# vniclas/VFM-Registration

Hardware: AMD Instinct MI355X
Metric: registrations/sec (20k<->200k pts, 384-D) (higher is better)
Workload: dtype fp6 (MX e2m3) coarse pass (scaled MFMA, fp32 scores + bounds from measured residuals) + int8 rescan (exact integer scores) + f32 refinement + f64 exact decision / f64 RANSAC

## Files before the change

include/vfmreg_debug.h:

```cpp
#ifndef VFMREG_DEBUG_H
#define VFMREG_DEBUG_H

#include "vfmreg.h"

#ifdef __cplusplus
extern "C" {
#endif

int vfm_prof_events_create(void **start, void **stop);
int vfm_prof_arm(void *start, void *stop);
int vfm_prof_elapsed_ms(void *start, void *stop, float *ms_host);
int vfm_prof_events_destroy(void *start, void *stop);

int vfm_debug_last_coarse_kernel(char *buf_host, int cap);
int vfm_debug_coarse_kernel_names(char *buf_host, int cap);

int vfm_debug_search_plan(int records, int d, int64_t n, int64_t m, int gated, char *buf_host, int cap);

int vfm_debug_coarse_plan(int records, int d, int64_t n, int64_t m, int gated, int inner_product, int row_bias, int compute_units,
                          char *buf_host, int cap);

enum vfm_debug_prepare_entry {
    VFM_PREP_ENTRY_PREPARE = 0,
    VFM_PREP_ENTRY_PREPARE2,
    VFM_PREP_ENTRY_GATED,
    VFM_PREP_ENTRY_GATED_P,
    VFM_PREP_ENTRY_GATED_Z,
    VFM_PREP_ENTRY_GATED_T,
    VFM_PREP_ENTRY_PERM,
    VFM_PREP_ENTRY_ONESHOT
};
int vfm_debug_prepare_plan(int entry, int schedule, int d, int64_t rows1, int dtype1, int64_t rows2, int dtype2, int zero, char *buf_host,
                           int cap);

int vfm_debug_match_stats(void *ws, int64_t n, int64_t m, int32_t *out64_host);
int vfm_debug_voxel_trace(void *ws, int64_t n, int64_t *out_host);
int vfm_debug_i8_rows(const void *prepared, int64_t rows, int d, int8_t *q8_host, float *step_host,
                      float *err_host, float *gerr_host);
int vfm_debug_mx6_rows(const void *prepared, int64_t rows, int d, float *v6_host, float *err_host, float *gerr_host);
int vfm_debug_mx6_half_err(const void *prepared, int64_t rows, int d, float *errh_host, float *gerrh_host);
int vfm_debug_ransac_counts(const void *ws, int64_t c_max, int32_t n_iter, int32_t *out_host);
#define VFM_DEBUG_RANSAC_CAND_MAX 2048
int vfm_debug_ransac_state(const void *ws, int64_t c_max, int32_t n_iter, int32_t *n_lo_host, int32_t *n_hi_host, double *r_lo_host,
                           double *r_hi_host, int32_t *sel_host, double *rstar_host, int32_t *list_host, double *fit_host,
                           double *rmse_host, int32_t *hyp_host);

int vfm_debug_vit_workspace_layout(const vfm_vit_config *cfg, int B, int64_t *offsets_host, int64_t *bytes_host);

int vfm_debug_vit_plan(const vfm_vit_config *cfg, int B, int W, int compute_units, char *buf_host, int cap);

int vfm_debug_l2_narrow_slices(int64_t n, int64_t m);
int vfm_debug_l2_narrow_evals(const void *ws, int64_t *out2_host);

#ifdef __cplusplus
}
#endif
#endif
```

vfm-registration_amd/csrc/config.cpp:

```cpp
#include "common.h"
#include "config.h"

#include <string.h>

#include <new>

struct vfm_config {
    VfmConfig c;
};

static const VfmConfig k_factory{};
static thread_local const VfmConfig* t_bound = nullptr;

const VfmConfig& vfm_cfg() { return t_bound ? *t_bound : k_factory; }

namespace {
struct Field {
    const char* name;
    int VfmConfig::*p;
};
const Field k_fields[] = {
    {"coarse_slices", &VfmConfig::force_slices},     {"match_stats", &VfmConfig::match_stats},
    {"i8_min_queries", &VfmConfig::i8_min_queries},  {"prep_grid", &VfmConfig::prep_grid},
    {"ransac_exact_only", &VfmConfig::ransac_exact_only}, {"ransac_fused", &VfmConfig::ransac_fused},
    {"coarse_qsets", &VfmConfig::coarse_qsets},      {"seed_units", &VfmConfig::seed_units},
    {"select_variant", &VfmConfig::select_variant},  {"mx6_t4", &VfmConfig::mx6_t4},
    {"mx6_tune", &VfmConfig::mx6_tune},
    {"mx6_ns3", &VfmConfig::mx6_ns3},                {"prep_form", &VfmConfig::prep_form},
    {"finish_short", &VfmConfig::finish_short},      {"rescan_rows", &VfmConfig::rescan_rows},
    {"half_noi8", &VfmConfig::half_noi8},            {"rescore_block", &VfmConfig::rescore_block},
    {"vit_preprocess_patch", &VfmConfig::vit_preprocess_patch}, {"vit_xcd", &VfmConfig::vit_xcd},
    {"vit_cfg_narrow", &VfmConfig::vit_cfg_narrow},  {"vit_cfg_wide", &VfmConfig::vit_cfg_wide},
    {"vit_wpw", &VfmConfig::vit_wpw},                {"vit_hot_a", &VfmConfig::vit_hot_a},
    {"vit_wide_tile", &VfmConfig::vit_wide_tile},    {"vit_lds_shape", &VfmConfig::vit_lds_shape},
    {"vit_att_lds_min", &VfmConfig::vit_att_lds_min}, {"vit_lds_min_wg", &VfmConfig::vit_lds_min_wg},
    {"vit_astat_min", &VfmConfig::vit_astat_min},    {"vit_astat_two", &VfmConfig::vit_astat_two},
    {"vit_astat_nw", &VfmConfig::vit_astat_nw},      {"vit_fused_qkv", &VfmConfig::vit_fused_qkv},
    {"vit_trace_fused", &VfmConfig::vit_trace_fused},  {"vit_fused_mlp", &VfmConfig::vit_fused_mlp},
    {"voxel_replay2", &VfmConfig::voxel_replay2},    {"voxel_one_launch", &VfmConfig::voxel_small},
    {"voxel_trace", &VfmConfig::voxel_trace},        {"voxel_grid_ppt", &VfmConfig::voxel_grid_ppt},
};

const char* const k_trace_buffer = "vit_trace_buffer";

void set_coarse_variant(VfmConfig& c, int v) {
    if (v == 60 || v == 61) { c.rescan_rows = v == 61 ? 1 : 0; return; }
    if (v == 50 || v == 51) { c.finish_short = v == 51 ? 1 : 0; return; }
    if (v >= 40 && v <= 44) { c.prep_form = v == 44 ? 4 : v == 43 ? 3 : v == 41 ? 1 : 0; return; }
    if (v == 32 || v == 33) { c.mx6_ns3 = v == 33 ? 1 : 0; return; }
    if (v == 30 || v == 31) { c.mx6_t4 = v == 30 ? 1 : 0; return; }
    c.seed_units = v == 7 ? 0 : 1;
    if (v == 7) v = 0;
    c.select_variant = v == 20 ? 1 : (v == 21 ? 2 : 0);
    if (v == 20 || v == 21) v = 0;
    c.coarse_qsets = v;
}
void set_voxel_small(VfmConfig& c, int on) {
    if (on == 2 || on == 3) c.voxel_replay2 = on == 3;
    else if (on >= 10 && on <= 10 + 64) c.voxel_grid_ppt = on - 10;
    else if (on == 100 || on == 101) c.voxel_trace = on - 100;
    else c.voxel_small = on;
}
}

VFM_EXPORT int vfm_config_create(vfm_config_t** out) {
    VFM_CHECK_ARG(out, "config_create: null pointer");
    *out = new (std::nothrow) vfm_config();
    if (!*out) return vfm_fail(VFM_EINVAL, "config_create: out of memory");
    return VFM_OK;
}
VFM_EXPORT int vfm_config_destroy(vfm_config_t* cfg) {
    if (cfg && t_bound == &cfg->c) t_bound = nullptr;
    delete cfg;
    return VFM_OK;
}
VFM_EXPORT int vfm_config_use(const vfm_config_t* cfg) {
    t_bound = cfg ? &cfg->c : nullptr;
    return VFM_OK;
}
VFM_EXPORT int vfm_config_set(vfm_config_t* cfg, const char* key, int64_t value) {
    VFM_CHECK_ARG(cfg && key, "config_set: null pointer");
    if ((!strcmp(key, "coarse_variant") && value == 42) || (!strcmp(key, "prep_form") && value == 2))
        return vfm_fail(VFM_EINVAL, "config_set: %s %lld (fp6 operand preparation by width) has been removed", key, (long long)value);
    if (!strcmp(key, "rescore_block") && value != 64 && value != 256)
        return vfm_fail(VFM_EINVAL, "config_set: rescore_block %lld (a workgroup of match_rescore_kernel owns 64 or 256 queries)", (long long)value);
    if (!strcmp(key, "coarse_variant")) { set_coarse_variant(cfg->c, (int)value); return VFM_OK; }
    if (!strcmp(key, "voxel_small")) { set_voxel_small(cfg->c, (int)value); return VFM_OK; }
    if (!strcmp(key, k_trace_buffer)) { cfg->c.vit_astat_dbg = reinterpret_cast<unsigned long long*>((uintptr_t)value); return VFM_OK; }
    for (const Field& f : k_fields)
        if (!strcmp(key, f.name)) {
            cfg->c.*(f.p) = (int)value;
            return VFM_OK;
        }
    return vfm_fail(VFM_EINVAL, "config_set: unknown key '%s'", key);
}
VFM_EXPORT int vfm_config_get(const vfm_config_t* cfg, const char* key, int64_t* value) {
    VFM_CHECK_ARG(key && value, "config_get: null pointer");
    const VfmConfig& c = cfg ? cfg->c : vfm_cfg();
    if (!strcmp(key, k_trace_buffer)) { *value = (int64_t)(uintptr_t)c.vit_astat_dbg; return VFM_OK; }
    for (const Field& f : k_fields)
        if (!strcmp(key, f.name)) {
            *value = c.*(f.p);
            return VFM_OK;
        }
    return vfm_fail(VFM_EINVAL, "config_get: unknown key '%s'", key);
}
```

vfm-registration_amd/csrc/config.h:

```cpp
#pragma once

struct VfmConfig {
    int force_slices = 0;
    int coarse_qsets = 0;
    int seed_units = 1;
    int select_variant = 0;
    int mx6_t4 = 1;
    int mx6_ns3 = 1;
    int prep_form = 3;
    int finish_short = 0;
    int half_noi8 = 1;
    int rescore_block = 0;
    int rescan_rows = 1;
    int mx6_tune = 0;
    int match_stats = 0;
    int i8_min_queries = 0;
    int prep_grid = -1;
    int ransac_exact_only = 0;
    int ransac_fused = 2;
    int vit_preprocess_patch = 1, vit_xcd = 1, vit_cfg_narrow = 108, vit_cfg_wide = 108, vit_wpw = 0, vit_hot_a = 0, vit_wide_tile = 0,
        vit_lds_shape = 23, vit_att_lds_min = 1, vit_lds_min_wg = 256, vit_astat_min = 0, vit_astat_two = 1, vit_astat_nw = 0,
        vit_trace_fused = 0,
        vit_fused_mlp = 0,
        vit_fused_qkv = 0;
    unsigned long long* vit_astat_dbg = nullptr;
    int voxel_replay2 = 1, voxel_small = 1, voxel_trace = 0, voxel_grid_ppt = 0;
};

const VfmConfig& vfm_cfg();
```

vfm-registration_amd/csrc/ransac.hip:

```cpp
#include <string.h>

#include <atomic>
#include <vector>

#include "../../include/vfmreg_debug.h"
#include "common.h"
#include "rot3.h"

namespace {

__device__ __forceinline__ void philox4x32_10(uint32_t c0, uint32_t c1, uint32_t c2, uint32_t c3, uint32_t k0,
                                              uint32_t k1, uint32_t out[4]) {
    const uint32_t M0 = 0xD2511F53u, M1 = 0xCD9E8D57u, W0 = 0x9E3779B9u, W1 = 0xBB67AE85u;
#pragma unroll
    for (int r = 0; r < 10; ++r) {
        const uint32_t hi0 = __umulhi(M0, c0), lo0 = M0 * c0;
        const uint32_t hi1 = __umulhi(M1, c2), lo1 = M1 * c2;
        const uint32_t n0 = hi1 ^ c1 ^ k0;
        const uint32_t n1 = lo1;
        const uint32_t n2 = hi0 ^ c3 ^ k1;
        const uint32_t n3 = lo0;
        c0 = n0; c1 = n1; c2 = n2; c3 = n3;
        k0 += W0; k1 += W1;
    }
    out[0] = c0; out[1] = c1; out[2] = c2; out[3] = c3;
}

__device__ bool kabsch_rows(const double* A, const double* B, const double* w, int64_t n, double denom_eps,
                            double T[12]) {
    double ma[3] = {0.0, 0.0, 0.0}, mb[3] = {0.0, 0.0, 0.0}, sw = 0.0;
    for (int64_t i = 0; i < n; ++i) {
        const double wi = w ? w[i] : 1.0;
        sw = sw + wi;
#pragma unroll
        for (int c = 0; c < 3; ++c) {
            ma[c] = ma[c] + wi * A[i * 3 + c];
            mb[c] = mb[c] + wi * B[i * 3 + c];
        }
    }
// ... 431 lines not shown
    __shared__ double red[6][1024];
    __shared__ double cen[6];
    const int64_t C = count_dev ? min(*count_dev, c_max) : c_max;
    if (threadIdx.x == 0) {
        sel->F = 0;
        sel->count = 0;
        sel->Rbits = 0x7FF0000000000000ull;
        sel->overflow = 0;
        sel->unsure = 0;
        sel->done = 0;
    }
    for (int64_t i = threadIdx.x; i < C; i += 1024) {
        int64_t a = corres[2 * i], b = corres[2 * i + 1];
        if (bad_out && (a < 0 || a >= ns || b < 0 || b >= nt)) {
            *bad_out = 1;
            a = b = 0;
        }
#pragma unroll
        for (int c = 0; c < 3; ++c) {
            pts[6 * i + c] = src[3 * a + c];
            pts[6 * i + 3 + c] = tgt[3 * b + c];
        }
    }
    __threadfence();
    __syncthreads();
    ransac_center_body(pts, C, stats, pts32, red, cen);
}

struct CoarseHyp {
    int32_t n_lo, n_hi;
    double r_lo, r_hi;
};

__global__ __launch_bounds__(64) void ransac_moment_kernel(const double* __restrict__ pts, const RansacStats* __restrict__ stats,
                                                           const int64_t* __restrict__ count_dev, int64_t c_max,
                                                           double max_d2, int32_t n_iter, uint64_t seed,
                                                           CoarseHyp* __restrict__ out, SelectState* __restrict__ sel, int rfuse) {
    const int64_t C = count_dev ? min(*count_dev, c_max) : c_max;
    const int lane = threadIdx.x;
    const int32_t h = (int32_t)(blockIdx.x * 64 + lane);
    CoarseHyp o = CoarseHyp{0, -1, 0.0, 0.0};
    bool unsure = false, sure_live = false;
    if (C >= 3 && h < n_iter) {
        double T[12];
        if (sample_T(pts, C, (uint32_t)h, seed, T)) {
            const double u = 1.1102230246251565e-16;
            double tau[3], taumax = 0.0, tt = 0.0, tabs = 0.0, rmax = 0.0;
#pragma unroll
            for (int r = 0; r < 3; ++r) {
                tau[r] = (T[4 * r + 3] + ((T[4 * r] * stats->cs[0] + T[4 * r + 1] * stats->cs[1]) + T[4 * r + 2] * stats->cs[2])) -
                         stats->cq[r];
                taumax = fmax(taumax, fabs(tau[r]));
                tt += tau[r] * tau[r];
                tabs = fmax(tabs, fabs(T[4 * r + 3]));
#pragma unroll
                for (int c = 0; c < 3; ++c) rmax = fmax(rmax, fabs(T[4 * r + c]));
            }
            const double reach = 4.01 * stats->M + taumax;
            const bool sure = (rmax <= 1.001) && (max_d2 > 0.0) && (3.0 * reach * reach * 1.001 < max_d2);
            if (!sure) {
                unsure = true;
            } else {
                const double* S = stats->Sss;
                double q1 = 0.0, rk = 0.0, t4 = 0.0;
#pragma unroll
                for (int a = 0; a < 3; ++a) {
                    const double x = T[4 * a], y = T[4 * a + 1], z = T[4 * a + 2];
                    q1 += (x * (S[0] * x + S[1] * y + S[2] * z) + y * (S[1] * x + S[3] * y + S[4] * z)) +
                          z * (S[2] * x + S[4] * y + S[5] * z);
                    rk += (x * stats->K[3 * a] + y * stats->K[3 * a + 1]) + z * stats->K[3 * a + 2];
                    t4 += tau[a] * (((x * stats->sbar[0] + y * stats->sbar[1]) + z * stats->sbar[2]) - stats->kbar[a]);
                }
                const double Cd = (double)C;
// ... 401 lines not shown
                sr[0] = sr[w];
                sh[0] = sh[w];
            }
        double T[12] = {1, 0, 0, 0, 0, 1, 0, 0, 0, 0, 1, 0};
        if (sh[0] >= 0) sample_T(pts, C, (uint32_t)sh[0], seed, T);
        for (int k = 0; k < 12; ++k) {
            T_out[k] = T[k];
            Ts[k] = T[k];
        }
        T_out[12] = 0.0;
        T_out[13] = 0.0;
        T_out[14] = 0.0;
        T_out[15] = 1.0;
        *fitness_out = (sh[0] >= 0) ? sf[0] : 0.0;
        *rmse_out = (sh[0] >= 0) ? sr[0] : 0.0;
        *best_hyp_out = sh[0];
    }
    __syncthreads();
    if (!mask) return;
    const bool have = sh[0] >= 0;
    double T[12];
#pragma unroll
    for (int k = 0; k < 12; ++k) T[k] = Ts[k];
    for (int64_t i = threadIdx.x; i < c_max; i += 1024) {
        uint8_t m = 0;
        if (i < C && have) {
            const double* p = pts + 6 * i;
            m = (err2(T, p[0], p[1], p[2], p[3], p[4], p[5]) < max_d2) ? 1 : 0;
        }
        mask[i] = m;
    }
}

__global__ __launch_bounds__(64) void ransac_exact_list_kernel(const double* __restrict__ pts,
                                                               const int64_t* __restrict__ count_dev, int64_t c_max,
                                                               double max_d2, int32_t n_iter, uint64_t seed,
                                                               const int32_t* __restrict__ list,
                                                               const SelectState* __restrict__ sel,
                                                               HypScore* __restrict__ best_out) {
    __shared__ __attribute__((aligned(16))) double d2s[EXACT_CHUNK];
    const int64_t C = count_dev ? min(*count_dev, c_max) : c_max;
    const int lane = threadIdx.x;
    HypScore res;
    res.fit = 0.0;
    res.rmse = 0.0;
    res.hyp = -1;
    const int ncand = sel->overflow ? 0 : min(sel->count, CAND_MAX);
    if ((int)blockIdx.x < ncand && C >= 3) {
        const int32_t h = list[blockIdx.x];
        double T[12];
        if (sample_T(pts, C, (uint32_t)h, seed, T)) {
            int64_t good = 0;
            double e2 = 0.0;
            for (int64_t base = 0; base < C; base += EXACT_CHUNK) {
                const int cnt = (int)min((int64_t)EXACT_CHUNK, C - base);
                __builtin_amdgcn_wave_barrier();
                int mine = 0;
                for (int i = lane; i < cnt; i += 64) {
                    const double* p = pts + 6 * (base + i);
                    const double d2 = err2(T, p[0], p[1], p[2], p[3], p[4], p[5]);
                    const bool in = d2 < max_d2;
                    mine += in ? 1 : 0;
                    d2s[i] = in ? d2 : 0.0;
                }
#pragma unroll
                for (int off = 32; off >= 1; off >>= 1) mine += __shfl_xor(mine, off);
                good += mine;
                __builtin_amdgcn_wave_barrier();
                int i = 0;
                if (cnt >= 32) {
                    double va[16], vb[16];
#pragma unroll
                    for (int u = 0; u < 16; ++u) va[u] = d2s[u];
                    for (; i + 48 <= cnt; i += 32) {
#pragma unroll
                        for (int u = 0; u < 16; ++u) vb[u] = d2s[i + 16 + u];
#pragma unroll
                        for (int u = 0; u < 16; ++u) e2 = e2 + va[u];
#pragma unroll
                        for (int u = 0; u < 16; ++u) va[u] = d2s[i + 32 + u];
#pragma unroll
                        for (int u = 0; u < 16; ++u) e2 = e2 + vb[u];
                    }
#pragma unroll
                    for (int u = 0; u < 16; ++u) e2 = e2 + va[u];
                    i += 16;
                }
                for (; i < cnt; ++i) e2 = e2 + d2s[i];
            }
            if (good > 0) {
                res.fit = (double)good / (double)C;
                res.rmse = sqrt(e2 / (double)good);
                res.hyp = h;
            }
        }
    }
    if (lane == 0) best_out[blockIdx.x] = res;
}

struct RansacWs {
    double* pts;
    float* pts32;
    RansacStats* stats;
    CoarseHyp* hyps;
    int32_t* list;
    SelectState* sel;
    HypScore* block_best;
    size_t bytes;
};
inline RansacWs carve_ransac(void* p, int64_t c_max, int32_t n_iter) {
    VfmCarver c(p);
    RansacWs w;
    w.pts = c.take<double>((size_t)(c_max > 0 ? c_max : 1) * 6);
    w.pts32 = c.take<float>((size_t)(c_max > 0 ? c_max : 1) * 6 + 4);
    w.stats = c.take<RansacStats>(1);
    w.hyps = c.take<CoarseHyp>((size_t)n_iter);
    w.list = c.take<int32_t>(CAND_MAX);
    w.sel = c.take<SelectState>(1);
    w.block_best = c.take<HypScore>((size_t)(n_iter + 63) / 64 + CAND_MAX + 1);
    w.bytes = c.used();
    return w;
}


}


VFM_EXPORT int vfm_debug_ransac_counts(const void* ws, int64_t c_max, int32_t n_iter, int32_t* out_host) {
    VFM_CHECK_ARG(ws && out_host && c_max >= 0 && n_iter > 0, "ransac_counts: bad arguments");
    RansacWs w = carve_ransac(const_cast<void*>(ws), c_max, n_iter);
// ... 13 lines not shown
    RansacWs w = carve_ransac(const_cast<void*>(ws), c_max, n_iter);
    SelectState s;
    VFM_CHECK_HIP(hipMemcpy(&s, w.sel, sizeof(s), hipMemcpyDeviceToHost));
    if (sel_host) {
        sel_host[0] = s.F;
        sel_host[1] = s.count;
        sel_host[2] = s.overflow;
        sel_host[3] = s.unsure;
    }
    if (rstar_host) memcpy(rstar_host, &s.Rbits, sizeof(double));
    if (n_lo_host || n_hi_host || r_lo_host || r_hi_host) {
        std::vector<CoarseHyp> hy((size_t)n_iter);
        VFM_CHECK_HIP(hipMemcpy(hy.data(), w.hyps, sizeof(CoarseHyp) * hy.size(), hipMemcpyDeviceToHost));
        for (int32_t h = 0; h < n_iter; ++h) {
            if (n_lo_host) n_lo_host[h] = hy[h].n_lo;
            if (n_hi_host) n_hi_host[h] = hy[h].n_hi;
            if (r_lo_host) r_lo_host[h] = hy[h].r_lo;
            if (r_hi_host) r_hi_host[h] = hy[h].r_hi;
        }
    }
    if (list_host) {
        const int n = s.count < 0 ? 0 : (s.count < CAND_MAX ? s.count : CAND_MAX);
        if (n > 0) VFM_CHECK_HIP(hipMemcpy(list_host, w.list, sizeof(int32_t) * (size_t)n, hipMemcpyDeviceToHost));
    }
    if (fit_host || rmse_host || hyp_host) {
        std::vector<HypScore> bb((size_t)CAND_MAX + (size_t)((n_iter + 63) / 64));
        VFM_CHECK_HIP(hipMemcpy(bb.data(), w.block_best, sizeof(HypScore) * bb.size(), hipMemcpyDeviceToHost));
        for (size_t k = 0; k < bb.size(); ++k) {
            if (fit_host) fit_host[k] = bb[k].fit;
            if (rmse_host) rmse_host[k] = bb[k].rmse;
            if (hyp_host) hyp_host[k] = bb[k].hyp;
        }
    }
    return VFM_OK;
}

VFM_EXPORT size_t vfm_ransac_workspace_bytes(int64_t c_max, int32_t n_iter) { return carve_ransac(nullptr, c_max, n_iter).bytes; }

namespace {
int ransac_corr_impl(const double* src, int64_t ns, const double* tgt, int64_t nt, const int32_t* corres, const int64_t* count_dev,
                     int64_t c_max, double max_dist, int32_t n_iter, uint64_t seed, double* T_out, double* fitness_out,
                     double* rmse_out, uint8_t* inlier_mask, int32_t* best_hyp_out, int32_t* bad_out, void* ws, size_t ws_bytes,
                     vfm_stream_t stream);
}
VFM_EXPORT int vfm_ransac_corr(const double* src, const double* tgt, const int32_t* corres, const int64_t* count_dev,
                               int64_t c_max, double max_dist, int32_t n_iter, uint64_t seed, double* T_out,
                               double* fitness_out, double* rmse_out, uint8_t* inlier_mask, int32_t* best_hyp_out,
                               void* ws, size_t ws_bytes, vfm_stream_t stream) {
    return ransac_corr_impl(src, 0, tgt, 0, corres, count_dev, c_max, max_dist, n_iter, seed, T_out, fitness_out, rmse_out, inlier_mask,
                            best_hyp_out, nullptr, ws, ws_bytes, stream);
}
VFM_EXPORT int vfm_ransac_corr_bounded(const double* src, int64_t ns, const double* tgt, int64_t nt, const int32_t* corres,
                                       const int64_t* count_dev, int64_t c_max, double max_dist, int32_t n_iter, uint64_t seed,
                                       double* T_out, double* fitness_out, double* rmse_out, uint8_t* inlier_mask,
                                       int32_t* best_hyp_out, int32_t* bad_out, void* ws, size_t ws_bytes, vfm_stream_t stream) {
    VFM_CHECK_ARG(bad_out && ns > 0 && nt > 0, "ransac: bad_out / cloud sizes");
    return ransac_corr_impl(src, ns, tgt, nt, corres, count_dev, c_max, max_dist, n_iter, seed, T_out, fitness_out, rmse_out, inlier_mask,
                            best_hyp_out, bad_out, ws, ws_bytes, stream);
}
namespace {
int ransac_corr_impl(const double* src, int64_t ns, const double* tgt, int64_t nt, const int32_t* corres, const int64_t* count_dev,
                     int64_t c_max, double max_dist, int32_t n_iter, uint64_t seed, double* T_out, double* fitness_out,
                     double* rmse_out, uint8_t* inlier_mask, int32_t* best_hyp_out, int32_t* bad_out, void* ws, size_t ws_bytes,
                     vfm_stream_t stream) {
    VFM_CHECK_ARG(src && tgt && corres && T_out && fitness_out && rmse_out && best_hyp_out && ws, "ransac: null pointer");
    VFM_CHECK_ARG(c_max >= 0 && n_iter > 0, "ransac: bad sizes (c_max=%lld n_iter=%d)", (long long)c_max, n_iter);
// ... 4 lines not shown
    const int nblocks = (n_iter + 63) / 64;
    if (vfm_cfg().ransac_fused == 1 && !vfm_cfg().ransac_exact_only && c_max > 0) {
        const int cus = vfm_compute_units();
        hipLaunchKernelGGL(ransac_prepare_kernel, dim3(1), dim3(1024), 0, st, src, tgt, corres, count_dev, c_max, w.pts, ns, nt, bad_out,
                           w.stats, w.pts32, w.sel);
        hipLaunchKernelGGL(ransac_moment_kernel, dim3(nblocks), dim3(64), 0, st, w.pts, w.stats, count_dev, c_max, max_d2, n_iter, seed,
                           w.hyps, w.sel, 1);
        hipLaunchKernelGGL(ransac_coarse_loop_kernel, dim3(nblocks < cus ? nblocks : cus), dim3(64 * COARSE_WAVES), 0, st, w.pts, w.pts32,
                           w.stats, count_dev, c_max, max_dist, n_iter, seed, w.hyps, w.sel);
        hipLaunchKernelGGL(ransac_select_exact_kernel, dim3(nblocks), dim3(64), 0, st, w.pts, count_dev, c_max, max_d2, n_iter, seed,
                           w.hyps, w.sel, w.block_best + CAND_MAX);
        VFM_CHECK_LAUNCH("ransac fused chain");
        hipLaunchKernelGGL(ransac_final_mask_kernel, dim3(1), dim3(1024), 0, st, w.pts, count_dev, c_max, max_d2, seed,
                           w.block_best + CAND_MAX, nblocks, T_out, fitness_out, rmse_out, best_hyp_out, inlier_mask);
        VFM_CHECK_LAUNCH("ransac_final_mask_kernel");
        return VFM_OK;
    }
    if (c_max > 0) {
        hipLaunchKernelGGL(ransac_gather_kernel, dim3((unsigned)((c_max + 255) / 256)), dim3(256), 0, st, src, tgt, corres,
                           count_dev, c_max, w.pts, ns, nt, bad_out);
        VFM_CHECK_LAUNCH("ransac_gather_kernel");
    }
    if (vfm_cfg().ransac_exact_only) {
        hipLaunchKernelGGL(ransac_score_kernel, dim3(nblocks), dim3(64), 0, st, w.pts, count_dev, c_max, max_d2, n_iter, seed,
                           (const int32_t*)nullptr, w.block_best);
        VFM_CHECK_LAUNCH("ransac_score_kernel");
        hipLaunchKernelGGL(ransac_final_kernel, dim3(1), dim3(256), 0, st, w.pts, count_dev, c_max, seed, w.block_best,
                           nblocks, T_out, fitness_out, rmse_out, best_hyp_out);
    } else {
        const unsigned gsel = (unsigned)((n_iter + 255) / 256);
        if (vfm_cfg().ransac_fused == 2) {
            const int cus = vfm_compute_units();
            hipLaunchKernelGGL(ransac_center_kernel, dim3(1), dim3(1024), 0, st, w.pts, count_dev, c_max, w.stats, w.pts32, w.sel);
            hipLaunchKernelGGL(ransac_moment_kernel, dim3(nblocks), dim3(64), 0, st, w.pts, w.stats, count_dev, c_max, max_d2,
                               n_iter, seed, w.hyps, w.sel, 1);
            hipLaunchKernelGGL(ransac_coarse_loop_kernel, dim3(nblocks < cus ? nblocks : cus), dim3(64 * COARSE_WAVES), 0, st, w.pts, w.pts32,
                               w.stats, count_dev, c_max, max_dist, n_iter, seed, w.hyps, w.sel);
            hipLaunchKernelGGL(ransac_select_list_kernel, dim3(gsel), dim3(256), 0, st, w.hyps, n_iter, w.sel, w.list);
            hipLaunchKernelGGL(ransac_exact_list_kernel, dim3(CAND_MAX), dim3(64), 0, st, w.pts, count_dev, c_max, max_d2, n_iter,
                               seed, w.list, w.sel, w.block_best);
            hipLaunchKernelGGL(ransac_score_kernel, dim3(nblocks), dim3(64), 0, st, w.pts, count_dev, c_max, max_d2, n_iter, seed,
                               &w.sel->overflow, w.block_best + CAND_MAX);
            VFM_CHECK_LAUNCH("ransac coarse/select/score kernels");
            hipLaunchKernelGGL(ransac_final_mask_kernel, dim3(1), dim3(1024), 0, st, w.pts, count_dev, c_max, max_d2, seed, w.block_best,
                               CAND_MAX + nblocks, T_out, fitness_out, rmse_out, best_hyp_out, c_max > 0 ? inlier_mask : (uint8_t*)nullptr);
            VFM_CHECK_LAUNCH("ransac_final_mask_kernel");
            return VFM_OK;
        }
        hipLaunchKernelGGL(ransac_sel_init_kernel, dim3(1), dim3(1), 0, st, w.sel);
        hipLaunchKernelGGL(ransac_center_kernel, dim3(1), dim3(1024), 0, st, w.pts, count_dev, c_max, w.stats, w.pts32, (SelectState*)nullptr);
        hipLaunchKernelGGL(ransac_moment_kernel, dim3(nblocks), dim3(64), 0, st, w.pts, w.stats, count_dev, c_max, max_d2,
                           n_iter, seed, w.hyps, w.sel, 0);
        hipLaunchKernelGGL(ransac_coarse_kernel, dim3(nblocks), dim3(64 * COARSE_WAVES), 0, st, w.pts, w.pts32, w.stats, count_dev, c_max,
                           max_dist, n_iter, seed, w.hyps, w.sel);
        hipLaunchKernelGGL(ransac_select_rmin_kernel, dim3(gsel), dim3(256), 0, st, w.hyps, n_iter, w.sel);
        hipLaunchKernelGGL(ransac_select_list_kernel, dim3(gsel), dim3(256), 0, st, w.hyps, n_iter, w.sel, w.list);
        hipLaunchKernelGGL(ransac_exact_list_kernel, dim3(CAND_MAX), dim3(64), 0, st, w.pts, count_dev, c_max, max_d2, n_iter,
                           seed, w.list, w.sel, w.block_best);
        hipLaunchKernelGGL(ransac_score_kernel, dim3(nblocks), dim3(64), 0, st, w.pts, count_dev, c_max, max_d2, n_iter, seed,
                           &w.sel->overflow, w.block_best + CAND_MAX);
        VFM_CHECK_LAUNCH("ransac coarse/select/score kernels");
        hipLaunchKernelGGL(ransac_final_kernel, dim3(1), dim3(256), 0, st, w.pts, count_dev, c_max, seed, w.block_best,
                           CAND_MAX + nblocks, T_out, fitness_out, rmse_out, best_hyp_out);
    }
    VFM_CHECK_LAUNCH("ransac_final_kernel");
    if (inlier_mask && c_max > 0) {
        hipLaunchKernelGGL(ransac_mask_kernel, dim3((unsigned)((c_max + 255) / 256)), dim3(256), 0, st, w.pts, count_dev,
                           c_max, max_d2, T_out, best_hyp_out, inlier_mask);
        VFM_CHECK_LAUNCH("ransac_mask_kernel");
    }
    return VFM_OK;
}
}

VFM_EXPORT int vfm_kabsch_batched(const double* A, const double* B, const double* w, int64_t b, int64_t n,
                                  double denom_eps, double* T_out, int32_t* valid, vfm_stream_t stream) {
    VFM_CHECK_ARG(A && B && T_out && b >= 0 && n >= 1, "kabsch: bad arguments");
    if (b == 0) return VFM_OK;
    hipLaunchKernelGGL(kabsch_batched_kernel, dim3((unsigned)((b + 63) / 64)), dim3(64), 0, (hipStream_t)stream, A, B, w, b,
                       n, denom_eps, T_out, valid);
    VFM_CHECK_LAUNCH("kabsch_batched_kernel");
    return VFM_OK;
}
```

vfm-registration_amd/vfmreg/_lib.py:

```python
from __future__ import annotations

import ctypes as C
from pathlib import Path

_HERE = Path(__file__).resolve().parent
LIB_PATH = _HERE / "lib" / "libvfmreg_hip.so"
_lib = None

c_i64 = C.c_int64
c_vp = C.c_void_p


class VitConfig(C.Structure):
    _fields_ = [("dim", C.c_int), ("depth", C.c_int), ("heads", C.c_int), ("mlp_dim", C.c_int),
                ("patch", C.c_int), ("patch_h", C.c_int), ("patch_w", C.c_int)]


class LiftCamera(C.Structure):
    _fields_ = [("mode", C.c_int), ("mats", C.c_double * 48), ("fc", C.c_double * 4), ("subsample", C.c_double),
                ("win", C.c_int64 * 4), ("H", C.c_int64), ("W", C.c_int64), ("proj_image", C.c_void_p),
                ("grid", C.c_void_p), ("raw_image", C.c_void_p), ("gh", C.c_int), ("gw", C.c_int), ("Hup", C.c_int),
                ("Wup", C.c_int), ("rot_mode", C.c_int)]


# ... 115 lines not shown
                                 C.c_size_t, c_vp]),
    "vfm_teaser_tls_translation_host": (C.c_int, [c_vp, c_i64, C.c_double, c_vp, c_vp]),
    "vfm_pca_moments_workspace_bytes": (C.c_size_t, [C.c_int]),
    "vfm_pca_moments": (C.c_int, [c_vp, C.c_int, c_i64, C.c_int, c_vp, c_vp, c_vp, C.c_size_t, c_vp]),
    "vfm_pca_project_workspace_bytes": (C.c_size_t, []),
    "vfm_pca_project": (C.c_int, [c_vp, C.c_int, c_i64, C.c_int, c_vp, c_vp, C.c_int, c_vp, c_vp, c_vp, c_vp, c_vp, C.c_size_t, c_vp]),
    "vfm_pca_colours": (C.c_int, [c_vp, c_vp, c_i64, C.c_int, c_vp, c_vp, c_vp, c_vp, c_vp]),
    "vfm_colour_gate": (C.c_int, [c_vp, c_i64, c_vp, C.c_int, C.c_double, c_vp, c_vp, c_vp]),
    "vfm_vit_weights_bytes": (C.c_size_t, [C.POINTER(VitConfig)]),
    "vfm_vit_weights_layout": (C.c_int, [C.POINTER(VitConfig), C.POINTER(c_i64), C.POINTER(c_i64), C.c_int]),
    "vfm_vit_workspace_bytes": (C.c_size_t, [C.POINTER(VitConfig), C.c_int]),
    "vfm_vit_forward": (C.c_int, [C.POINTER(VitConfig), c_vp, c_vp, C.c_int, C.c_int, C.c_int, c_vp, c_vp,
                                  C.c_size_t, c_vp]),
}


DEBUG_SIGNATURES = {
    "vfm_prof_events_create": (C.c_int, [C.POINTER(c_vp), C.POINTER(c_vp)]),
    "vfm_prof_arm": (C.c_int, [c_vp, c_vp]),
    "vfm_prof_elapsed_ms": (C.c_int, [c_vp, c_vp, C.POINTER(C.c_float)]),
    "vfm_prof_events_destroy": (C.c_int, [c_vp, c_vp]),
    "vfm_debug_last_coarse_kernel": (C.c_int, [C.c_char_p, C.c_int]),
    "vfm_debug_coarse_kernel_names": (C.c_int, [C.c_char_p, C.c_int]),
    "vfm_debug_search_plan": (C.c_int, [C.c_int, C.c_int, c_i64, c_i64, C.c_int, C.c_char_p, C.c_int]),
    "vfm_debug_coarse_plan": (C.c_int, [C.c_int, C.c_int, c_i64, c_i64, C.c_int, C.c_int, C.c_int, C.c_int, C.c_char_p, C.c_int]),
    "vfm_debug_prepare_plan": (C.c_int, [C.c_int, C.c_int, C.c_int, c_i64, C.c_int, c_i64, C.c_int, C.c_int, C.c_char_p, C.c_int]),
    "vfm_debug_match_stats": (C.c_int, [c_vp, c_i64, c_i64, c_vp]),
    "vfm_debug_i8_rows": (C.c_int, [c_vp, c_i64, C.c_int, c_vp, c_vp, c_vp, c_vp]),
    "vfm_debug_mx6_rows": (C.c_int, [c_vp, c_i64, C.c_int, c_vp, c_vp, c_vp]),
    "vfm_debug_mx6_half_err": (C.c_int, [c_vp, c_i64, C.c_int, c_vp, c_vp]),
    "vfm_debug_voxel_trace": (C.c_int, [c_vp, c_i64, c_vp]),
    "vfm_debug_ransac_counts": (C.c_int, [c_vp, c_i64, C.c_int, c_vp]),
    "vfm_debug_ransac_state": (C.c_int, [c_vp, c_i64, C.c_int, c_vp, c_vp, c_vp, c_vp, c_vp, c_vp, c_vp, c_vp, c_vp, c_vp]),
    "vfm_debug_vit_workspace_layout": (C.c_int, [C.POINTER(VitConfig), C.c_int, C.POINTER(c_i64), C.POINTER(c_i64)]),
    "vfm_debug_vit_plan": (C.c_int, [C.POINTER(VitConfig), C.c_int, C.c_int, C.c_int, C.c_char_p, C.c_int]),
    "vfm_debug_l2_narrow_slices": (C.c_int, [c_i64, c_i64]),
    "vfm_debug_l2_narrow_evals": (C.c_int, [c_vp, C.POINTER(c_i64)]),
}


def load() -> C.CDLL:
    global _lib
    if _lib is not None:
        return _lib
    if not LIB_PATH.exists():
        raise RuntimeError(
            f"{LIB_PATH} is missing: build it with `python vfm-registration_amd/build.py` "
            "(hipcc --offload-arch=gfx950). There is no CPU fallback.")
    import torch
    lib = C.CDLL(str(LIB_PATH))
    for name, (res, args) in list(SIGNATURES.items()) + list(DEBUG_SIGNATURES.items()):
        fn = getattr(lib, name)
        fn.restype = res
        fn.argtypes = args
    _install_tool_names(lib)
    _lib = lib
    return lib


import threading as _threading

_tls = _threading.local()


class Config:

# ... 137 lines not shown
```

Baseline: 2143.

## Replace serial f64 inlier-error sum with bit-exact wave scan in RANSAC exact scoring

The exact RANSAC candidate scoring used to sum squared inlier errors as one sequential f64 chain per hypothesis. It now computes the same left-to-right sum as a parallel wave scan over composable increment maps, falling back to the serial chain when the scan cannot guarantee identical rounding. The exact-list kernel also becomes a grid-stride loop over candidates with a smaller fixed grid, and the moment kernel launches 512-thread workgroups instead of 64. The scan adds per-chunk shuffle and ballot work and a fallback path, and the smaller grid may under-fill the GPU when there are many candidates.

```diff
diff --git a/include/vfmreg_debug.h b/include/vfmreg_debug.h
--- a/include/vfmreg_debug.h
+++ b/include/vfmreg_debug.h
@@ -44,6 +44,8 @@
 int vfm_debug_ransac_state(const void *ws, int64_t c_max, int32_t n_iter, int32_t *n_lo_host, int32_t *n_hi_host, double *r_lo_host,
                            double *r_hi_host, int32_t *sel_host, double *rstar_host, int32_t *list_host, double *fit_host,
                            double *rmse_host, int32_t *hyp_host);
+int vfm_debug_inorder_sum(const double *x_dev, int64_t n, double *sum_dev, int32_t *scan_blocks_dev, vfm_stream_t stream);
+int vfm_debug_inorder_sum_host(const double *x, int64_t n, double *sum, int32_t *scan_blocks);
 
 int vfm_debug_vit_workspace_layout(const vfm_vit_config *cfg, int B, int64_t *offsets_host, int64_t *bytes_host);
 
diff --git a/vfm-registration_amd/csrc/config.cpp b/vfm-registration_amd/csrc/config.cpp
--- a/vfm-registration_amd/csrc/config.cpp
+++ b/vfm-registration_amd/csrc/config.cpp
@@ -23,6 +23,7 @@
     {"coarse_slices", &VfmConfig::force_slices},     {"match_stats", &VfmConfig::match_stats},
     {"i8_min_queries", &VfmConfig::i8_min_queries},  {"prep_grid", &VfmConfig::prep_grid},
     {"ransac_exact_only", &VfmConfig::ransac_exact_only}, {"ransac_fused", &VfmConfig::ransac_fused},
+    {"ransac_sum", &VfmConfig::ransac_sum},          {"ransac_moment_block", &VfmConfig::ransac_moment_block},
     {"coarse_qsets", &VfmConfig::coarse_qsets},      {"seed_units", &VfmConfig::seed_units},
     {"select_variant", &VfmConfig::select_variant},  {"mx6_t4", &VfmConfig::mx6_t4},
     {"mx6_tune", &VfmConfig::mx6_tune},
@@ -84,6 +85,10 @@
         return vfm_fail(VFM_EINVAL, "config_set: %s %lld (fp6 operand preparation by width) has been removed", key, (long long)value);
     if (!strcmp(key, "rescore_block") && value != 64 && value != 256)
         return vfm_fail(VFM_EINVAL, "config_set: rescore_block %lld (a workgroup of match_rescore_kernel owns 64 or 256 queries)", (long long)value);
+    if (!strcmp(key, "ransac_moment_block") && value != 64 && value != 512)
+        return vfm_fail(VFM_EINVAL, "config_set: ransac_moment_block %lld (a workgroup of ransac_moment_kernel owns 64 or 512 hypotheses)", (long long)value);
+    if (!strcmp(key, "ransac_sum") && value != 0 && value != 1)
+        return vfm_fail(VFM_EINVAL, "config_set: ransac_sum %lld (1 = the in-order sum as a wave scan, 0 = as one chain)", (long long)value);
     if (!strcmp(key, "coarse_variant")) { set_coarse_variant(cfg->c, (int)value); return VFM_OK; }
     if (!strcmp(key, "voxel_small")) { set_voxel_small(cfg->c, (int)value); return VFM_OK; }
     if (!strcmp(key, k_trace_buffer)) { cfg->c.vit_astat_dbg = reinterpret_cast<unsigned long long*>((uintptr_t)value); return VFM_OK; }
diff --git a/vfm-registration_amd/csrc/config.h b/vfm-registration_amd/csrc/config.h
--- a/vfm-registration_amd/csrc/config.h
+++ b/vfm-registration_amd/csrc/config.h
@@ -18,6 +18,8 @@
     int prep_grid = -1;
     int ransac_exact_only = 0;
     int ransac_fused = 2;
+    int ransac_sum = 1;
+    int ransac_moment_block = 0;
     int vit_preprocess_patch = 1, vit_xcd = 1, vit_cfg_narrow = 108, vit_cfg_wide = 108, vit_wpw = 0, vit_hot_a = 0, vit_wide_tile = 0,
         vit_lds_shape = 23, vit_att_lds_min = 1, vit_lds_min_wg = 256, vit_astat_min = 0, vit_astat_two = 1, vit_astat_nw = 0,
         vit_trace_fused = 0,
diff --git a/vfm-registration_amd/csrc/inorder_sum.h b/vfm-registration_amd/csrc/inorder_sum.h
--- /dev/null
+++ b/vfm-registration_amd/csrc/inorder_sum.h
@@ -0,0 +1,167 @@
+#pragma once
+
+#include <stdint.h>
+
+#if defined(__HIPCC__)
+#define VFM_INORDER_HD __host__ __device__ __forceinline__
+#else
+#define VFM_INORDER_HD inline
+#endif
+
+constexpr int INORDER_RUN = 16;
+constexpr int INORDER_BLOCK = 64;
+constexpr int INORDER_CHUNK = 64 * INORDER_RUN;
+constexpr int INORDER_LANES_PER_BLOCK = INORDER_BLOCK / INORDER_RUN;
+constexpr int INORDER_STAGE = INORDER_CHUNK + INORDER_CHUNK / INORDER_RUN;
+VFM_INORDER_HD int inorder_slot(int i) { return i + (i >> 4); }
+
+constexpr uint64_t INORDER_MANT = (1ull << 52) - 1ull;
+constexpr uint64_t INORDER_ONE = 1ull << 52;
+constexpr uint64_t INORDER_LIMIT = 1ull << 53;
+
+struct InorderMap {
+    uint64_t inc0, inc1;
+};
+
+VFM_INORDER_HD uint64_t inorder_bits(double v) { return __builtin_bit_cast(uint64_t, v); }
+VFM_INORDER_HD double inorder_from_bits(uint64_t b) { return __builtin_bit_cast(double, b); }
+
+VFM_INORDER_HD bool inorder_scannable(double S) { return (inorder_bits(S) >> 52) - (1023ull - 900ull) <= 1800ull; }
+
+struct InorderRun {
+    double even, odd;
+    uint64_t sign;
+};
+VFM_INORDER_HD void inorder_run_begin(InorderRun& r, double S) {
+    const uint64_t base = inorder_bits(S) & ~INORDER_MANT;
+    r.even = inorder_from_bits(base);
+    r.odd = inorder_from_bits(base + 1ull);
+    r.sign = 0ull;
+}
+VFM_INORDER_HD void inorder_run_add(InorderRun& r, double x) {
+    r.even = r.even + x;
+    r.odd = r.odd + x;
+    r.sign |= inorder_bits(x);
+}
+VFM_INORDER_HD InorderMap inorder_run_end(const InorderRun& r, double S) {
+    const uint64_t base = inorder_bits(S) & ~INORDER_MANT;
+    InorderMap m;
+    m.inc0 = inorder_bits(r.even) - base;
+    m.inc1 = inorder_bits(r.odd) - (base + 1ull);
+    const bool refuse = (r.sign >> 63) != 0ull || m.inc0 > INORDER_ONE || m.inc1 > INORDER_ONE;
+    if (refuse) m.inc0 = m.inc1 = INORDER_LIMIT;
+    return m;
+}
+VFM_INORDER_HD InorderMap inorder_compose(const InorderMap& f, const InorderMap& g) {
+    InorderMap r;
+    r.inc0 = f.inc0 + ((f.inc0 & 1ull) ? g.inc1 : g.inc0);
+    r.inc1 = f.inc1 + ((f.inc1 & 1ull) ? g.inc0 : g.inc1);
+    return r;
+}
+VFM_INORDER_HD uint64_t inorder_apply(const InorderMap m, double S) {
+    const uint64_t s = (inorder_bits(S) & INORDER_MANT) | INORDER_ONE;
+    return s + (m.inc0 ^ ((m.inc0 ^ m.inc1) & (0ull - (s & 1ull))));
+}
+VFM_INORDER_HD bool inorder_accept(uint64_t t) { return t <= INORDER_LIMIT; }
+VFM_INORDER_HD double inorder_value(uint64_t t, double S) { return inorder_from_bits((inorder_bits(S) & ~INORDER_MANT) + (t - INORDER_ONE)); }
+
+inline double inorder_sum_host(const double* x, int64_t n, int32_t* scan_blocks) {
+    double S = 0.0;
+    int blocks = 0;
+    double xs[INORDER_STAGE];
+    for (int64_t base = 0; base < n; base += INORDER_CHUNK) {
+        const int cnt = (int)((n - base) < INORDER_CHUNK ? (n - base) : INORDER_CHUNK);
+        const int nblk = (cnt + INORDER_BLOCK - 1) / INORDER_BLOCK;
+        for (int i = 0; i < nblk * INORDER_BLOCK; ++i) xs[inorder_slot(i)] = i < cnt ? x[base + i] : 0.0;
+        int blk = 0;
+        while (blk < nblk) {
+            if (inorder_scannable(S)) {
+                InorderMap pre = InorderMap{0ull, 0ull};
+                int fb = nblk;
+                uint64_t t_keep = 0ull;
+                for (int lane = blk * INORDER_LANES_PER_BLOCK; lane < nblk * INORDER_LANES_PER_BLOCK; ++lane) {
+                    InorderRun r;
+                    inorder_run_begin(r, S);
+                    const double* p = xs + inorder_slot(lane * INORDER_RUN);
+                    for (int j = 0; j < INORDER_RUN; ++j) inorder_run_add(r, p[j]);
+                    pre = inorder_compose(pre, inorder_run_end(r, S));
+                    const uint64_t t = inorder_apply(pre, S);
+                    if (!inorder_accept(t)) {
+                        fb = lane / INORDER_LANES_PER_BLOCK;
+                        break;
+                    }
+                    if ((lane + 1) % INORDER_LANES_PER_BLOCK == 0) t_keep = t;
+                }
+                if (fb > blk) {
+                    S = inorder_value(t_keep, S);
+                    blocks += fb - blk;
+                    blk = fb;
+                }
+                if (blk >= nblk) break;
+            }
+            const double* p = xs + inorder_slot(blk * INORDER_BLOCK);
+            for (int q = 0; q < INORDER_LANES_PER_BLOCK; ++q)
+                for (int j = 0; j < INORDER_RUN; ++j) S = S + p[q * (INORDER_RUN + 1) + j];
+            ++blk;
+        }
+    }
+    if (scan_blocks) *scan_blocks = blocks;
+    return S;
+}
+
+#if defined(__HIPCC__)
+struct InorderWave {
+    __device__ __forceinline__ int lane() const { return (int)(threadIdx.x & 63u); }
+    __device__ __forceinline__ void scan(InorderMap& m) const {
+        const int l = lane();
+#pragma unroll
+        for (int d = 1; d < 64; d <<= 1) {
+            InorderMap o;
+            o.inc0 = __shfl_up((unsigned long long)m.inc0, (unsigned)d);
+            o.inc1 = __shfl_up((unsigned long long)m.inc1, (unsigned)d);
+            if (l >= d) m = inorder_compose(o, m);
+        }
+    }
+    __device__ __forceinline__ int first_refusing(bool refuse) const {
+        const unsigned long long b = __ballot(refuse);
+        return b ? __ffsll((long long)b) - 1 : 64;
+    }
+    __device__ __forceinline__ uint64_t take(uint64_t v, int src) const { return (uint64_t)__shfl((unsigned long long)v, src); }
+};
+__device__ __forceinline__ double inorder_wave_sum(double S, const double* xs, int cnt, int* scan_blocks) {
+    InorderWave w;
+    const int nblk = (cnt + INORDER_BLOCK - 1) / INORDER_BLOCK;
+    int blk = 0;
+    while (blk < nblk) {
+        if (inorder_scannable(S)) {
+            const int lane = w.lane();
+            InorderMap m = InorderMap{0ull, 0ull};
+            if (lane >= blk * INORDER_LANES_PER_BLOCK && lane < nblk * INORDER_LANES_PER_BLOCK) {
+                InorderRun r;
+                inorder_run_begin(r, S);
+                const double* p = xs + inorder_slot(lane * INORDER_RUN);
+#pragma unroll
+                for (int j = 0; j < INORDER_RUN; ++j) inorder_run_add(r, p[j]);
+                m = inorder_run_end(r, S);
+            }
+            w.scan(m);
+            const uint64_t t = inorder_apply(m, S);
+            int fb = w.first_refusing(!inorder_accept(t)) / INORDER_LANES_PER_BLOCK;
+            if (fb > nblk) fb = nblk;
+            if (fb > blk) {
+                S = inorder_value(w.take(t, fb * INORDER_LANES_PER_BLOCK - 1), S);
+                *scan_blocks += fb - blk;
+                blk = fb;
+            }
+            if (blk >= nblk) break;
+        }
+        const double* p = xs + inorder_slot(blk * INORDER_BLOCK);
+#pragma unroll
+        for (int q = 0; q < INORDER_LANES_PER_BLOCK; ++q)
+#pragma unroll
+            for (int j = 0; j < INORDER_RUN; ++j) S = S + p[q * (INORDER_RUN + 1) + j];
+        ++blk;
+    }
+    return S;
+}
+#endif
diff --git a/vfm-registration_amd/csrc/ransac.hip b/vfm-registration_amd/csrc/ransac.hip
--- a/vfm-registration_amd/csrc/ransac.hip
+++ b/vfm-registration_amd/csrc/ransac.hip
@@ -5,6 +5,7 @@
 
 #include "../../include/vfmreg_debug.h"
 #include "common.h"
+#include "inorder_sum.h"
 #include "rot3.h"
 
 namespace {
@@ -502,13 +503,13 @@
     double r_lo, r_hi;
 };
 
-__global__ __launch_bounds__(64) void ransac_moment_kernel(const double* __restrict__ pts, const RansacStats* __restrict__ stats,
+__global__ __launch_bounds__(512) void ransac_moment_kernel(const double* __restrict__ pts, const RansacStats* __restrict__ stats,
                                                            const int64_t* __restrict__ count_dev, int64_t c_max,
                                                            double max_d2, int32_t n_iter, uint64_t seed,
                                                            CoarseHyp* __restrict__ out, SelectState* __restrict__ sel, int rfuse) {
     const int64_t C = count_dev ? min(*count_dev, c_max) : c_max;
-    const int lane = threadIdx.x;
-    const int32_t h = (int32_t)(blockIdx.x * 64 + lane);
+    const int lane = threadIdx.x & 63;
+    const int32_t h = (int32_t)(blockIdx.x * blockDim.x + threadIdx.x);
     CoarseHyp o = CoarseHyp{0, -1, 0.0, 0.0};
     bool unsure = false, sure_live = false;
     if (C >= 3 && h < n_iter) {
@@ -976,70 +977,103 @@
     }
 }
 
+template <bool SCAN>
 __global__ __launch_bounds__(64) void ransac_exact_list_kernel(const double* __restrict__ pts,
                                                                const int64_t* __restrict__ count_dev, int64_t c_max,
                                                                double max_d2, int32_t n_iter, uint64_t seed,
                                                                const int32_t* __restrict__ list,
                                                                const SelectState* __restrict__ sel,
                                                                HypScore* __restrict__ best_out) {
-    __shared__ __attribute__((aligned(16))) double d2s[EXACT_CHUNK];
+    static_assert(EXACT_CHUNK == INORDER_CHUNK, "a staged chunk is one call of inorder_wave_sum");
+    __shared__ __attribute__((aligned(16))) double d2s[SCAN ? INORDER_STAGE : EXACT_CHUNK];
     const int64_t C = count_dev ? min(*count_dev, c_max) : c_max;
     const int lane = threadIdx.x;
-    HypScore res;
-    res.fit = 0.0;
-    res.rmse = 0.0;
-    res.hyp = -1;
     const int ncand = sel->overflow ? 0 : min(sel->count, CAND_MAX);
-    if ((int)blockIdx.x < ncand && C >= 3) {
-        const int32_t h = list[blockIdx.x];
-        double T[12];
-        if (sample_T(pts, C, (uint32_t)h, seed, T)) {
-            int64_t good = 0;
-            double e2 = 0.0;
-            for (int64_t base = 0; base < C; base += EXACT_CHUNK) {
-                const int cnt = (int)min((int64_t)EXACT_CHUNK, C - base);
-                __builtin_amdgcn_wave_barrier();
-                int mine = 0;
-                for (int i = lane; i < cnt; i += 64) {
-                    const double* p = pts + 6 * (base + i);
-                    const double d2 = err2(T, p[0], p[1], p[2], p[3], p[4], p[5]);
-                    const bool in = d2 < max_d2;
-                    mine += in ? 1 : 0;
-                    d2s[i] = in ? d2 : 0.0;
+    for (int slot = (int)blockIdx.x; slot < CAND_MAX; slot += (int)gridDim.x) {
+        HypScore res;
+        res.fit = 0.0;
+        res.rmse = 0.0;
+        res.hyp = -1;
+        if (slot < ncand && C >= 3) {
+            const int32_t h = list[slot];
+            double T[12];
+            if (sample_T(pts, C, (uint32_t)h, seed, T)) {
+                int64_t good = 0;
+                double e2 = 0.0;
+                int scanned = 0;
+                for (int64_t base = 0; base < C; base += EXACT_CHUNK) {
+                    const int cnt = (int)min((int64_t)EXACT_CHUNK, C - base);
+                    __builtin_amdgcn_wave_barrier();
+                    int mine = 0;
+                    for (int i = lane; i < (SCAN ? (cnt + 63) / 64 * 64 : cnt); i += 64) {
+                        double v = 0.0;
+                        if (!SCAN || i < cnt) {
+                            const double* p = pts + 6 * (base + i);
+                            const double d2 = err2(T, p[0], p[1], p[2], p[3], p[4], p[5]);
+                            const bool in = d2 < max_d2;
+                            mine += in ? 1 : 0;
+                            v = in ? d2 : 0.0;
+                        }
+                        d2s[SCAN ? inorder_slot(i) : i] = v;
+                    }
+#pragma unroll
+                    for (int off = 32; off >= 1; off >>= 1) mine += __shfl_xor(mine, off);
+                    good += mine;
+                    __builtin_amdgcn_wave_barrier();
+                    if (SCAN) {
+                        e2 = inorder_wave_sum(e2, d2s, cnt, &scanned);
+                        continue;
+                    }
+                    int i = 0;
+                    if (cnt >= 32) {
+                        double va[16], vb[16];
+#pragma unroll
+                        for (int u = 0; u < 16; ++u) va[u] = d2s[u];
+                        for (; i + 48 <= cnt; i += 32) {
+#pragma unroll
+                            for (int u = 0; u < 16; ++u) vb[u] = d2s[i + 16 + u];
+#pragma unroll
+                            for (int u = 0; u < 16; ++u) e2 = e2 + va[u];
+#pragma unroll
+                            for (int u = 0; u < 16; ++u) va[u] = d2s[i + 32 + u];
+#pragma unroll
+                            for (int u = 0; u < 16; ++u) e2 = e2 + vb[u];
+                        }
+#pragma unroll
+                        for (int u = 0; u < 16; ++u) e2 = e2 + va[u];
+                        i += 16;
+                    }
+                    for (; i < cnt; ++i) e2 = e2 + d2s[i];
                 }
-#pragma unroll
-                for (int off = 32; off >= 1; off >>= 1) mine += __shfl_xor(mine, off);
-                good += mine;
-                __builtin_amdgcn_wave_barrier();
-                int i = 0;
-                if (cnt >= 32) {
-                    double va[16], vb[16];
-#pragma unroll
-                    for (int u = 0; u < 16; ++u) va[u] = d2s[u];
-                    for (; i + 48 <= cnt; i += 32) {
-#pragma unroll
-                        for (int u = 0; u < 16; ++u) vb[u] = d2s[i + 16 + u];
-#pragma unroll
-                        for (int u = 0; u < 16; ++u) e2 = e2 + va[u];
-#pragma unroll
-                        for (int u = 0; u < 16; ++u) va[u] = d2s[i + 32 + u];
-#pragma unroll
-                        for (int u = 0; u < 16; ++u) e2 = e2 + vb[u];
-                    }
-#pragma unroll
-                    for (int u = 0; u < 16; ++u) e2 = e2 + va[u];
-                    i += 16;
+                if (good > 0) {
+                    res.fit = (double)good / (double)C;
+                    res.rmse = sqrt(e2 / (double)good);
+                    res.hyp = h;
                 }
-                for (; i < cnt; ++i) e2 = e2 + d2s[i];
-            }
-            if (good > 0) {
-                res.fit = (double)good / (double)C;
-                res.rmse = sqrt(e2 / (double)good);
-                res.hyp = h;
-            }
-        }
-    }
-    if (lane == 0) best_out[blockIdx.x] = res;
+            }
+        }
+        if (lane == 0) best_out[slot] = res;
+    }
+}
+constexpr int EXACT_LIST_GRID = CAND_MAX < 128 ? CAND_MAX : 128;
+
+__global__ __launch_bounds__(64) void inorder_sum_debug_kernel(const double* __restrict__ x, int64_t n, double* __restrict__ sum_out,
+                                                               int32_t* __restrict__ scan_blocks_out) {
+    __shared__ __attribute__((aligned(16))) double xs[INORDER_STAGE];
+    const int lane = threadIdx.x;
+    double S = 0.0;
+    int scanned = 0;
+    for (int64_t base = 0; base < n; base += INORDER_CHUNK) {
+        const int cnt = (int)min((int64_t)INORDER_CHUNK, n - base);
+        __builtin_amdgcn_wave_barrier();
+        for (int i = lane; i < (cnt + 63) / 64 * 64; i += 64) xs[inorder_slot(i)] = i < cnt ? x[base + i] : 0.0;
+        __builtin_amdgcn_wave_barrier();
+        S = inorder_wave_sum(S, xs, cnt, &scanned);
+    }
+    if (lane == 0) {
+        *sum_out = S;
+        *scan_blocks_out = scanned;
+    }
 }
 
 struct RansacWs {
@@ -1119,6 +1153,18 @@
             if (hyp_host) hyp_host[k] = bb[k].hyp;
         }
     }
+    return VFM_OK;
+}
+
+VFM_EXPORT int vfm_debug_inorder_sum(const double* x_dev, int64_t n, double* sum_dev, int32_t* scan_blocks_dev, vfm_stream_t stream) {
+    VFM_CHECK_ARG(sum_dev && scan_blocks_dev && n >= 0 && (x_dev || n == 0), "inorder_sum: bad arguments");
+    hipLaunchKernelGGL(inorder_sum_debug_kernel, dim3(1), dim3(64), 0, (hipStream_t)stream, x_dev, n, sum_dev, scan_blocks_dev);
+    VFM_CHECK_LAUNCH("inorder_sum_debug_kernel");
+    return VFM_OK;
+}
+VFM_EXPORT int vfm_debug_inorder_sum_host(const double* x, int64_t n, double* sum, int32_t* scan_blocks) {
+    VFM_CHECK_ARG(sum && n >= 0 && (x || n == 0), "inorder_sum_host: bad arguments");
+    *sum = inorder_sum_host(x, n, scan_blocks);
     return VFM_OK;
 }
 
@@ -1189,13 +1235,18 @@
         if (vfm_cfg().ransac_fused == 2) {
             const int cus = vfm_compute_units();
             hipLaunchKernelGGL(ransac_center_kernel, dim3(1), dim3(1024), 0, st, w.pts, count_dev, c_max, w.stats, w.pts32, w.sel);
-            hipLaunchKernelGGL(ransac_moment_kernel, dim3(nblocks), dim3(64), 0, st, w.pts, w.stats, count_dev, c_max, max_d2,
-                               n_iter, seed, w.hyps, w.sel, 1);
+            const int mblock = vfm_cfg().ransac_moment_block == 64 ? 64 : 512;
+            hipLaunchKernelGGL(ransac_moment_kernel, dim3((unsigned)((n_iter + mblock - 1) / mblock)), dim3(mblock), 0, st, w.pts, w.stats,
+                               count_dev, c_max, max_d2, n_iter, seed, w.hyps, w.sel, 1);
             hipLaunchKernelGGL(ransac_coarse_loop_kernel, dim3(nblocks < cus ? nblocks : cus), dim3(64 * COARSE_WAVES), 0, st, w.pts, w.pts32,
                                w.stats, count_dev, c_max, max_dist, n_iter, seed, w.hyps, w.sel);
             hipLaunchKernelGGL(ransac_select_list_kernel, dim3(gsel), dim3(256), 0, st, w.hyps, n_iter, w.sel, w.list);
-            hipLaunchKernelGGL(ransac_exact_list_kernel, dim3(CAND_MAX), dim3(64), 0, st, w.pts, count_dev, c_max, max_d2, n_iter,
-                               seed, w.list, w.sel, w.block_best);
+            if (vfm_cfg().ransac_sum)
+                hipLaunchKernelGGL(ransac_exact_list_kernel<true>, dim3(EXACT_LIST_GRID), dim3(64), 0, st, w.pts, count_dev, c_max, max_d2,
+                                   n_iter, seed, w.list, w.sel, w.block_best);
+            else
+                hipLaunchKernelGGL(ransac_exact_list_kernel<false>, dim3(CAND_MAX), dim3(64), 0, st, w.pts, count_dev, c_max, max_d2,
+                                   n_iter, seed, w.list, w.sel, w.block_best);
             hipLaunchKernelGGL(ransac_score_kernel, dim3(nblocks), dim3(64), 0, st, w.pts, count_dev, c_max, max_d2, n_iter, seed,
                                &w.sel->overflow, w.block_best + CAND_MAX);
             VFM_CHECK_LAUNCH("ransac coarse/select/score kernels");
@@ -1212,7 +1263,7 @@
                            max_dist, n_iter, seed, w.hyps, w.sel);
         hipLaunchKernelGGL(ransac_select_rmin_kernel, dim3(gsel), dim3(256), 0, st, w.hyps, n_iter, w.sel);
         hipLaunchKernelGGL(ransac_select_list_kernel, dim3(gsel), dim3(256), 0, st, w.hyps, n_iter, w.sel, w.list);
-        hipLaunchKernelGGL(ransac_exact_list_kernel, dim3(CAND_MAX), dim3(64), 0, st, w.pts, count_dev, c_max, max_d2, n_iter,
+        hipLaunchKernelGGL(ransac_exact_list_kernel<false>, dim3(CAND_MAX), dim3(64), 0, st, w.pts, count_dev, c_max, max_d2, n_iter,
                            seed, w.list, w.sel, w.block_best);
         hipLaunchKernelGGL(ransac_score_kernel, dim3(nblocks), dim3(64), 0, st, w.pts, count_dev, c_max, max_d2, n_iter, seed,
                            &w.sel->overflow, w.block_best + CAND_MAX);
diff --git a/vfm-registration_amd/vfmreg/_lib.py b/vfm-registration_amd/vfmreg/_lib.py
--- a/vfm-registration_amd/vfmreg/_lib.py
+++ b/vfm-registration_amd/vfmreg/_lib.py
@@ -171,6 +171,8 @@
     "vfm_debug_voxel_trace": (C.c_int, [c_vp, c_i64, c_vp]),
     "vfm_debug_ransac_counts": (C.c_int, [c_vp, c_i64, C.c_int, c_vp]),
     "vfm_debug_ransac_state": (C.c_int, [c_vp, c_i64, C.c_int, c_vp, c_vp, c_vp, c_vp, c_vp, c_vp, c_vp, c_vp, c_vp, c_vp]),
+    "vfm_debug_inorder_sum": (C.c_int, [c_vp, c_i64, c_vp, c_vp, c_vp]),
+    "vfm_debug_inorder_sum_host": (C.c_int, [c_vp, c_i64, c_vp, c_vp]),
     "vfm_debug_vit_workspace_layout": (C.c_int, [C.POINTER(VitConfig), C.c_int, C.POINTER(c_i64), C.POINTER(c_i64)]),
     "vfm_debug_vit_plan": (C.c_int, [C.POINTER(VitConfig), C.c_int, C.c_int, C.c_int, C.c_char_p, C.c_int]),
     "vfm_debug_l2_narrow_slices": (C.c_int, [c_i64, c_i64]),
```

Result: no change. 2138 (-0.2%).
